# JessicaLeu-code/MotionPlanning_5D_m

Hardware: AMD Instinct MI355X
Metric: CFS iterations/sec, 5-DoF 30-wp 8-obs batch-1024; l_inf wp err vs quadprog (higher is better)
Workload: dtype f64

## Files before the change

### motionplanning_5d_m_amd/csrc/cfs_fused.hip

```cpp
#include "cfs_geom_dev.h"
#include <algorithm>
#include <atomic>

namespace {

#define STAMP(k) do { if (P.stamps) { const unsigned long long t_ = clock64(); if (tid == 0) s_acc[k] += t_ - t0_; t0_ = t_; } } while (0)

#ifndef CFS_CERT_AT
#define CFS_CERT_AT 6
#endif
constexpr int CERT_AT = CFS_CERT_AT;
#ifndef CFS_WG_PER_CU
#define CFS_WG_PER_CU 1
#endif
#ifndef CFS_ANGLE_ADD
#define CFS_ANGLE_ADD 0
#endif
#ifndef CFS_REF_A
#define CFS_REF_A 1e-4
#define CFS_REF_B 1e-9
#endif
#ifndef CFS_MV_BATCH
#define CFS_MV_BATCH 16
#endif
// ... 356 lines not shown
};
__host__ __device__ inline FusedLayout fused_layout(int NJ, int H, int nobs, int QB, int PR)
{
    FusedLayout L;
    const int HN = H * NJ, NS = 2 * NJ;
    int o = 0;
    L.rb = o; o += (int)(sizeof(DevRobot) / 8);
    L.ob = o; o += nobs * 6;
    L.x = o; o += H * NS;
    L.u = o; o += HN;
    L.qu = o; o += HN;
    L.g = o; o += nobs * HN;
    L.rhs = o; o += nobs * H;
    L.xs = o; o += 3 * HN;
    L.up = o; o += HN;
    L.act = o; o += (QB + 1) / 2;
    L.fre = o; o += (QB + 1) / 2;
    L.prev = o; o += (QB + 1) / 2;
    L.flag = o; o += (nobs * H + 4 * HN + 7) / 8;
    L.code = o; o += (nobs * H + 4 * HN + 1) / 2;
    L.red = o; o += 64;
    L.small = o; o += 4 * NJ + nobs;
    L.mx = o; o += HN;
    L.racc = o; o += HN;
    L.cost = o; o += (int)(sizeof(DevCost) / 8);
    o = (o + 1) & ~1;
    L.lin = o;
    L.wb = o; o += 3 * HN;
    L.zb = o; o += 3 * HN;
    L.d = o; o += QB;
    L.r = o; o += QB;
    L.rho = o; o += QB;
    L.lam = o; o += QB;
    L.prow = o; o += QB;
    L.slot = o; o += (nobs * H + 4 * HN + 3) / 4;
    L.ptail = o;
    o = (o + 1) & ~1;
    L.y = o;
    L.total_fixed = o;
    return L;
}

template <int NJ, int QB, bool IDENT>
__global__ __launch_bounds__(FT, CFS_WG_PER_CU) void CFS_FUSED_KERNEL(FusedParams P CFS_SOFT_KPARAM)
{
    constexpr int NS = 2 * NJ, NVT = nvt(NJ), NE = 2 * NJ + 1;
    extern __shared__ __attribute__((aligned(16))) double lds[];
    const int b = P.order ? P.order[blockIdx.x] : (int)blockIdx.x, tid = threadIdx.x;
    const int H = P.H, nobs = P.nobs, HN = H * NJ, nn = HN, NX = H * NS;
    const double dt = P.dt;
    constexpr int PR = QB < CFS_PR ? QB : CFS_PR;
    const FusedLayout L = fused_layout(NJ, H, nobs, QB, PR);
    DevRobot *rb = reinterpret_cast<DevRobot *>(lds + L.rb);
    double *s_ob = lds + L.ob, *s_x = lds + L.x, *s_u = lds + L.u, *s_qu = lds + L.qu, *s_g = lds + L.g;
    double *s_rhs = lds + L.rhs, *xs = lds + L.xs, *s_up = lds + L.up, *wb = lds + L.wb, *zb = lds + L.zb;
    double *s_d = lds + L.d, *s_r = lds + L.r, *s_rho = lds + L.rho, *s_lam = lds + L.lam, *s_prow = lds + L.prow;
    int *s_act = reinterpret_cast<int *>(lds + L.act);
    int *s_free = reinterpret_cast<int *>(lds + L.fre);
    int *s_prev = reinterpret_cast<int *>(lds + L.prev);
    unsigned char *s_flag = reinterpret_cast<unsigned char *>(lds + L.flag);
    unsigned short *s_slot = reinterpret_cast<unsigned short *>(lds + L.slot);
    int *s_code = reinterpret_cast<int *>(lds + L.code);
    double *red_base = lds + L.red;
    int red_sel = 0;
#define red (red_base + 24 * (red_sel ^= 1))
    double *s_lim = lds + L.small, *s_v0 = s_lim + NJ, *s_th0 = s_v0 + NJ, *s_margin = s_th0 + 2 * NJ;
    double *s_mx = lds + L.mx;
    double *s_racc = lds + L.racc;
    int pool_slot;
    {
        int *pubp = reinterpret_cast<int *>(red_base + 63);
        if (tid == 0) {
            int sidx = (int)(((blockIdx.x * 0x9E3779B1u) >> 8) % (unsigned)P.pool_n);
            int probes = 0;
            while (atomicCAS(&P.pool_flag[sidx * 16], 0, 1) != 0) {
                sidx = sidx + 1 == P.pool_n ? 0 : sidx + 1;
                __builtin_amdgcn_s_sleep(2);
                if (++probes > (1 << 22)) { sidx = -1; break; }
            }
            pubp[0] = sidx;
        }
        __syncthreads();
        pool_slot = pubp[0];
        if (pool_slot < 0) {
            if (tid == 0 && P.piece == 0) { P.status[b] = CFS_NUMERIC; P.iter_O[b] = 1; P.total_iter[b] = 0; }
            return;
        }
    }
    double *const s_pt = P.Pt + (size_t)pool_slot * P.pt_stride;
    double *s_Y = lds + L.y;
    const int QY = P.qy;
    double *const Yg = P.Yg + (size_t)pool_slot * nn * nn;
    auto drop_pool = [&]() {
        __syncthreads();
        if (tid == 0) { __threadfence(); atomicExch(&P.pool_flag[pool_slot * 16], 0); }
    };
    const int ncon = nobs * H + (P.has_bounds ? 4 : 2) * HN;
    const int maxit = 8 * nn + 200;
    for (int e = tid; e < ncon; e += FT) {
        int code;
        if (e < nobs * H) { const int j = e / H; code = mk_code(CT_COL, e - j * H, j); }
        else {
            const int f2 = e - nobs * H, ty = f2 / HN, k = f2 - ty * HN, i = k / NJ;
            code = mk_code(1 + ty, i, k - i * NJ);
        }
        s_code[e] = code;
    }

    {
        const double *src = reinterpret_cast<const double *>(P.rb);
        for (int e = tid; e < (int)(sizeof(DevRobot) / 8); e += FT) lds[L.rb + e] = src[e];
        for (int e = tid; e < nobs * 6; e += FT) s_ob[e] = P.obs[(size_t)b * nobs * 6 + e];
        for (int e = tid; e < NX; e += FT) s_x[e] = P.x_init[(size_t)b * NX + e];
        for (int e = tid; e < HN; e += FT) { s_u[e] = 0.0; s_qu[e] = 0.0; s_mx[e] = P.has_bounds ? P.maxin[e] : 0.0; }
        if (tid < NJ) {
            s_lim[tid] = P.lim[tid];
            s_v0[tid] = P.xR1[(size_t)b * NS + NJ + tid];
            s_th0[tid] = P.xR1[(size_t)b * NS + tid];
        }
        if (tid < nobs) s_margin[tid] = P.margin[tid];
        if (P.cost) {
            const double *csrc = reinterpret_cast<const double *>(P.cost);
            for (int e = tid; e < (int)(sizeof(DevCost) / 8); e += FT) lds[L.cost + e] = csrc[e];
        }
    }
    __syncthreads();
    if (P.has_bounds)
        for (int e = tid; e < HN; e += FT) {
            const int i = e / NJ, c = e - i * NJ;
            double acc = 0.0;
            for (int k = 0; k <= i; ++k) acc += ((double)(i - k) + 0.5) * s_mx[k * NJ + c];
            s_racc[e] = (dt * dt) * acc;
        }
    unsigned long long *s_acc = reinterpret_cast<unsigned long long *>(red_base + 48);
    if (tid < 12) s_acc[tid] = 0ull;
    unsigned long long t0_ = P.stamps ? clock64() : 0ull;
    double cost_new = P.caug[b], cost_old = 100000.0;
    int iter_O = 1, total_iter = 0, noise_row = 0, status = CFS_OK_MAXITER;
    bool done = false;
#if CFS_SOFT
    const double iw = S.inv_weight;
    int n_soft = 0;
    bool last_soft = false;
#endif
    const int nseg = nobs - P.nmesh;
    int launched = 0;
    if (P.resume) {
        for (int e = tid; e < NX; e += FT) s_x[e] = P.x_[(size_t)b * NX + e];
        for (int e = tid; e < HN; e += FT) { s_u[e] = P.u[(size_t)b * nn + e]; s_qu[e] = P.st_qu[(size_t)b * nn + e]; }
        cost_new = P.st_cost[2 * b]; cost_old = P.st_cost[2 * b + 1];
        iter_O = P.iter_O[b]; total_iter = P.total_iter[b]; status = P.status[b];
        noise_row = P.st_noise[b]; done = P.st_done[b] != 0;
        __syncthreads();
    } else if (P.piece == 0) {
        double d2 = 0.0;
        for (int e = tid; e < NX; e += FT) { const double v = s_x[e] - 1.0; d2 += v * v; }
        d2 = block_sum(d2, red, tid);
        if (sqrt(d2) < P.epsilon_O) { done = true; status = CFS_OK_CONVERGED; }
        else if (iter_O > P.max_o_iter) { done = true; status = CFS_OK_MAXITER; }
    } else if (P.piece == 2) {
        for (int e = tid; e < HN; e += FT) s_u[e] = P.u[(size_t)b * nn + e];
        __syncthreads();
    }

    PRow<PR, QB> Pr;
    int prev_q = 0;

    while (!done) {
        bool skip = false;
        if (P.piece == 0 && P.mode == CFS_MODE_PSGCFS) {
            skip = fabs(cost_new - cost_old) < 1e-4;
            if (!skip) cost_old = cost_new;
        } else if (P.piece == 0) cost_old = cost_new;
        const int noise_row_now = noise_row;
        if (P.piece == 0 && P.mode == CFS_MODE_PSGCFS && !skip) ++noise_row;
        auto prep = [&](int ph) {
            if (P.piece == 1) return;
            if (ph == 0) { for (int k = tid; k < HN; k += FT) xs[k] = s_u[k]; }
            else if (ph == 1) roll_lds<NJ>(xs, H, dt, tid);
            else if (ph == 2) {
                const bool psg = P.piece == 0 && P.mode == CFS_MODE_PSGCFS;
                const double sc = (double)iter_O * (double)iter_O + 1.0;
                const bool have = P.noise != nullptr && noise_row_now < P.noise_rows;
                for (int k = tid; k < HN; k += FT) {
                    s_up[k] = xs[2 * HN + k];
                    double v;
                    if (psg && skip) v = s_u[k];
                    else if (psg) {
                        const double nz = have ? P.noise[((size_t)b * P.noise_rows + noise_row_now) * nn + k] : 0.0;
                        v = s_u[k] - P.alpha * ((s_qu[k] + P.ff[(size_t)b * nn + k]) + 10.0 * nz / sc);
                    } else v = P.x0[(size_t)b * nn + k];
                    xs[k] = v;
                }
            } else roll_lds<NJ>(xs, H, dt, tid);
        };
        bool prepped = false;
#if CFS_JAC
        (void)NE;
        if (nseg > 0) {
            const int W = P.lin_w;
            double *s_sc = lds + L.lin;
            double *s_en = s_sc + W * NJ * 6;
            double *s_tw = s_en + W * NJ * 6;
            double *s_bd = s_en + W * NVT * 6;
            for (int w0 = 0; w0 < H; w0 += W) {
                const int Wc = min(W, H - w0);
                if (w0 == 0) prep(0);
                for (int e = tid; e < Wc * NJ; e += FT) {
                    const int m = e % NJ, wi = e / NJ;
                    double x = s_x[(w0 + wi) * NS + m];
                    x = x - rb->th_off[m];
                    double sn, cs;
                    sincos(x, &sn, &cs);
                    s_sc[e * 2] = sn;
                    s_sc[e * 2 + 1] = cs;
                }
                __syncthreads();
                for (int wi = tid; wi < Wc; wi += FT) arm_chain(rb, NJ, s_sc + wi * NJ * 2, s_en + wi * NJ * 6, s_tw + wi * NJ * 6);
                if (w0 == 0) prep(1);
                __syncthreads();
                STAMP(10);
                for (int e = tid; e < NJ * Wc * nseg; e += FT) {
                    const int j = e % nseg, wi = (e / nseg) % Wc, k0 = e / (nseg * Wc);
                    s_bd[(wi * NJ + k0) * nseg + j] = seg_seg_dist(s_en + (wi * NJ + k0) * 6, s_ob + j * 6);
                }
                if (w0 == 0) prep(2);
                __syncthreads();
                STAMP(0);
                for (int e = tid; e < Wc * nseg; e += FT) {
                    const int j = e % nseg, wi = e / nseg;
                    double m0 = INFINITY;
                    int lk = 0;
#pragma unroll
                    for (int k1 = 1; k1 <= NJ; ++k1) { const double bk = s_bd[(wi * NJ + k1 - 1) * nseg + j]; if (bk < m0) { m0 = bk; lk = k1; } }
                    if (P.dump_linkid && launched == 0) P.dump_linkid[((size_t)b * nobs + j) * H + w0 + wi] = lk;
                    s_rhs[j * H + w0 + wi] = m0;
                    double *g = s_g + (j * H + w0 + wi) * NJ;
                    if (lk > 0) winner_grad(s_en + (wi * NJ + lk - 1) * 6, s_tw + wi * NJ * 6, lk - 1, NJ, s_ob + j * 6, g);
                    else for (int m = 0; m < NJ; ++m) g[m] = 0.0;
                }
                if (w0 == 0) { prep(3); prepped = true; }
                if (w0 + W >= H) __syncthreads();
                STAMP(11);
            }
        }
#else
        if (nseg > 0) {
            const int W = P.lin_w;
            double *s_sc = lds + L.lin;
            double *s_en = s_sc + W * NJ * 6;
            double *s_bd = s_en + W * NVT * 6;
            double *s_dv = s_bd + W * NJ * nseg;
            unsigned short *s_list = reinterpret_cast<unsigned short *>(s_dv + W * nseg * NE);
            int *s_cnt = s_free;
            for (int w0 = 0; w0 < H; w0 += W) {
                const int Wc = min(W, H - w0);
                if (w0 == 0) prep(0);
#if CFS_ANGLE_ADD
                const double ch = cos(FD_EPS / 2), sh = sin(FD_EPS / 2);
                for (int e = tid; e < Wc * NJ; e += FT) {
                    const int m = e % NJ, wi = e / NJ;
                    double sn, cs;
                    sincos(s_x[(w0 + wi) * NS + m] - rb->th_off[m], &sn, &cs);
                    s_sc[e * 6] = sn;
                    s_sc[e * 6 + 1] = cs;
                    s_sc[e * 6 + 2] = sn * ch + cs * sh; s_sc[e * 6 + 3] = cs * ch - sn * sh;
                    s_sc[e * 6 + 4] = sn * ch - cs * sh; s_sc[e * 6 + 5] = cs * ch + sn * sh;
                }
#else
                for (int e = tid; e < Wc * NJ * 3; e += FT) {
                    const int var = e % 3, m = (e / 3) % NJ, wi = e / (3 * NJ);
                    double x = s_x[(w0 + wi) * NS + m];
                    if (var == 1) x = x + FD_EPS / 2;
                    else if (var == 2) x = x - FD_EPS / 2;
                    x = x - rb->th_off[m];
                    double sn, cs;
                    sincos(x, &sn, &cs);
                    s_sc[((wi * NJ + m) * 3 + var) * 2] = sn;
                    s_sc[((wi * NJ + m) * 3 + var) * 2 + 1] = cs;
                }
#endif
                __syncthreads();
                for (int e = tid; e < Wc * NE; e += FT) {
                    const int ev = e % NE, wi = e / NE;
                    double M[12], Mn[12], e6[6];
#pragma unroll
                    for (int k1 = 1; k1 <= NJ; ++k1) {
                        const int avar = (ev == 2 * k1 - 1) ? 1 : (ev >= 2 * k1 ? 2 : 0);
                        const double sn = s_sc[((wi * NJ + k1 - 1) * 3 + avar) * 2], cs = s_sc[((wi * NJ + k1 - 1) * 3 + avar) * 2 + 1];
                        fk_step(rb, k1 - 1, sn, cs, k1 == 1 ? nullptr : M, Mn);
#pragma unroll
                        for (int qq = 0; qq < 12; ++qq) M[qq] = Mn[qq];
                        if (ev <= 2 * k1) {
                            link_ends(rb, k1 - 1, M, e6);
                            double *dstE = s_en + (wi * NVT + kvoff(k1) + ev) * 6;
#pragma unroll
                            for (int qq = 0; qq < 6; ++qq) dstE[qq] = e6[qq];
                        }
                    }
                }
                if (w0 == 0) prep(1);
                __syncthreads();
                STAMP(10);
#if CFS_LIN_UNROLL
#pragma unroll 2
#endif
                for (int e = tid; e < NJ * Wc * nseg; e += FT) {
                    const int j = e % nseg, wi = (e / nseg) % Wc, k0 = e / (nseg * Wc);
                    s_bd[(wi * NJ + k0) * nseg + j] = seg_seg_dist(s_en + (wi * NVT + kvoff(k0 + 1)) * 6, s_ob + j * 6);
                }
                if (tid < NJ) s_cnt[tid] = 0;
                if (w0 == 0) prep(2);
                __syncthreads();
                for (int e = tid; e < Wc * nseg; e += FT) {
                    const int j = e % nseg, wi = e / nseg;
                    double bk[NJ], m0 = INFINITY;
                    int lk = 0;
#pragma unroll
                    for (int k1 = 1; k1 <= NJ; ++k1) { bk[k1 - 1] = s_bd[(wi * NJ + k1 - 1) * nseg + j]; if (bk[k1 - 1] < m0) { m0 = bk[k1 - 1]; lk = k1; } }
                    if (P.dump_linkid && launched == 0) P.dump_linkid[((size_t)b * nobs + j) * H + w0 + wi] = lk;
                    const double thr = P.no_prune ? INFINITY : fmax(m0, 0.0001) + rb->prune_tol;
#pragma unroll
                    for (int k1 = 1; k1 <= NJ; ++k1)
                        if (bk[k1 - 1] < thr) s_list[(k1 - 1) * W * nseg + atomicAdd(&s_cnt[k1 - 1], 1)] = (unsigned short)((wi << 8) | j);
                    s_dv[e * NE] = m0;
#pragma unroll
                    for (int ev = 1; ev < NE; ++ev) s_dv[e * NE + ev] = INFINITY;
                }
                if (w0 == 0) { prep(3); prepped = true; }
                __syncthreads();
                STAMP(0);
                {
                    int offs[NJ + 1];
                    offs[0] = 0;
#pragma unroll
                    for (int k1 = 1; k1 <= NJ; ++k1) offs[k1] = offs[k1 - 1] + s_cnt[k1 - 1] * 2 * k1;
#if CFS_LIN_UNROLL
#pragma unroll 2
#endif
                    for (int e = tid; e < offs[NJ]; e += FT) {
                        int k1 = 1, ent = 0, v = 1;
#pragma unroll
                        for (int kk = 1; kk <= NJ; ++kk)
                            if (e >= offs[kk - 1] && e < offs[kk]) {
                                const int r_ = e - offs[kk - 1];
                                k1 = kk; ent = r_ / (2 * kk); v = r_ - ent * (2 * kk) + 1;
                            }
                        const int item = s_list[(k1 - 1) * W * nseg + ent], wi = item >> 8, j = item & 255;
                        const double dis = seg_seg_dist(s_en + (wi * NVT + kvoff(k1) + v) * 6, s_ob + j * 6);
                        double *dv = s_dv + (wi * nseg + j) * NE;
                        const int evhi = (v == 2 * k1) ? NE - 1 : v;
                        for (int ev = v; ev <= evhi; ++ev)
                            __hip_atomic_fetch_min(dv + ev, dis, __ATOMIC_RELAXED, __HIP_MEMORY_SCOPE_WORKGROUP);
                    }
                }
                __syncthreads();
                STAMP(11);
                for (int e = tid; e < Wc * nseg; e += FT) {
                    const int j = e % nseg, wi = e / nseg;
                    double dev[NE];
#pragma unroll
                    for (int ev = 0; ev < NE; ++ev) dev[ev] = s_dv[e * NE + ev];
                    s_rhs[j * H + w0 + wi] = dev[0];
#pragma unroll
                    for (int m = 0; m < NJ; ++m) s_g[(j * H + w0 + wi) * NJ + m] = (dev[2 * m + 1] - dev[2 * m + 2]) / FD_EPS;
                }
                if (w0 + W >= H) __syncthreads();
            }
        }
#endif
        if (!prepped && P.piece != 1) {
            prep(0); __syncthreads(); prep(1); __syncthreads(); prep(2); __syncthreads(); prep(3); __syncthreads();
        }

        if (P.nmesh > 0) {
            for (int e = tid; e < P.nmesh * H; e += FT) s_rhs[nseg * H + e] = P.ext_dist[(size_t)b * P.nmesh * H + e];
            for (int e = tid; e < P.nmesh * HN; e += FT) s_g[nseg * HN + e] = P.ext_grad[(size_t)b * P.nmesh * HN + e];
            __syncthreads();
        }

        if (P.dump_dist && launched == 0) {
            for (int e = tid; e < nobs * H; e += FT) P.dump_dist[(size_t)b * nobs * H + e] = s_rhs[e];
            for (int e = tid; e < nobs * HN; e += FT) P.dump_grad[(size_t)b * nobs * HN + e] = s_g[e];
        }
        if (P.piece == 1) { drop_pool(); return; }

        STAMP(0);
        int qp_status = QP_OK, iters = 0;
        int qhi = 0, nfree = 0;
        int npolish = 0;
        auto n_combine = [&](const double *coef, const double *base, int pc_) {
            const int ptype_ = pc_ >> 16, pi_ = (pc_ >> 8) & 0xff, pj_ = pc_ & 0xff;
            const bool two = H <= 32;
            const int lane = two ? (tid & 31) : (tid & 63);
            const int iR = H - 1 - lane;
            const int cstep = two ? 2 * (FT / 64) : FT / 64;
            for (int c = two ? (tid >> 5) : (tid >> 6); c < NJ; c += cstep) {
                double Rp = 0.0, Rv = 0.0;
                if (lane < H) {
                    const int sp_ = s_slot[nobs * H + iR * NJ + c], sm_ = s_slot[nobs * H + HN + iR * NJ + c];
                    for (int j0 = 0; j0 < nobs; j0 += 8) {
                        int sl[8];
#pragma unroll
                        for (int jj = 0; jj < 8; ++jj) sl[jj] = j0 + jj < nobs ? s_slot[(j0 + jj) * H + iR] : 0;
#pragma unroll
                        for (int jj = 0; jj < 8; ++jj)
                            if (sl[jj]) Rp += coef[sl[jj] - 1] * s_g[((j0 + jj) * H + iR) * NJ + c];
                    }
                    if (sp_) Rv -= dt * coef[sp_ - 1];
                    if (sm_) Rv += dt * coef[sm_ - 1];
                }
                const double S1 = two ? half_scan_incl(Rp) : wave_scan_incl(Rp);
                const double cmb = (dt * dt) * S1 + Rv;
                const double S2V = two ? half_scan_incl(cmb) : wave_scan_incl(cmb);
                const double nr_rev = S2V - (0.5 * dt * dt) * S1;
                const int src = (lane < H ? H - 1 - lane : lane) + (two ? (tid & 32) : 0);
                const double nr = __shfl(nr_rev, src, 64);
                double z0 = 0.0;
                if (lane < H) {
                    if (base) z0 = base[lane * NJ + c];
                    else if (ptype_ == CT_COL) z0 = lane <= pi_ ? s_g[(pj_ * H + pi_) * NJ + c] * ((dt * dt) * ((double)(pi_ - lane) + 0.5)) : 0.0;
                    else z0 = (c == pj_ && lane <= pi_) ? (ptype_ == CT_VELP ? -dt : dt) : 0.0;
                    z0 -= nr;
                }
                const double sv = dt * (two ? half_scan_incl(z0) : wave_scan_incl(z0));
                const double spo = dt * (two ? half_scan_incl(sv) : wave_scan_incl(sv)) - (0.5 * dt) * sv;
                if (lane < H) { zb[lane * NJ + c] = z0; zb[HN + lane * NJ + c] = sv; zb[2 * HN + lane * NJ + c] = spo; }
            }
        };
        auto y_combine = [&](const double *coef, const double *base) {
            const int qa = min(qhi, QY);
            for (int k = tid; k < HN; k += FT) {
                double z0 = base ? base[k] : 0.0, z1 = 0.0, z2 = 0.0, z3 = 0.0;
                int a = 0;
                for (; a + 4 <= qa; a += 4) {
                    z0 -= coef[a] * s_Y[a * HN + k];
                    z1 -= coef[a + 1] * s_Y[(a + 1) * HN + k];
                    z2 -= coef[a + 2] * s_Y[(a + 2) * HN + k];
                    z3 -= coef[a + 3] * s_Y[(a + 3) * HN + k];
                }
                for (; a < qa; ++a) z0 -= coef[a] * s_Y[a * HN + k];
                for (a = qa; a + CFS_TU <= qhi; a += CFS_TU) {
                    double t[CFS_TU];
#pragma unroll
                    for (int jj = 0; jj < CFS_TU; ++jj) t[jj] = Yg[(size_t)(a + jj) * nn + k];
#pragma unroll
                    for (int jj = 0; jj < CFS_TU; jj += 4) {
                        z0 -= coef[a + jj] * t[jj]; z1 -= coef[a + jj + 1] * t[jj + 1]; z2 -= coef[a + jj + 2] * t[jj + 2]; z3 -= coef[a + jj + 3] * t[jj + 3];
                    }
                }
                for (; a < qhi; ++a) z0 -= coef[a] * Yg[(size_t)a * nn + k];
                zb[k] = (z0 + z1) + (z2 + z3);
            }
        };
        auto y_combine_roll = [&](const double *coef, const double *base) {
            const int lane = tid & 31;
            for (int c = tid >> 5; c < NJ; c += 2 * (FT / 64)) {
                const int k = lane * NJ + c;
                double z0 = 0.0, z1 = 0.0, z2 = 0.0, z3 = 0.0;
                if (lane < H) {
                    z0 = base ? base[k] : 0.0;
                    int a = 0;
                    for (; a + 4 <= qhi; a += 4) {
                        z0 -= coef[a] * s_Y[a * HN + k];
                        z1 -= coef[a + 1] * s_Y[(a + 1) * HN + k];
                        z2 -= coef[a + 2] * s_Y[(a + 2) * HN + k];
                        z3 -= coef[a + 3] * s_Y[(a + 3) * HN + k];
                    }
                    for (; a < qhi; ++a) z0 -= coef[a] * s_Y[a * HN + k];
                }
                const double z = (z0 + z1) + (z2 + z3);
                const double sv = dt * half_scan_incl(z);
                const double spo = dt * half_scan_incl(sv) - (0.5 * dt) * sv;
                if (lane < H) { zb[k] = z; zb[HN + k] = sv; zb[2 * HN + k] = spo; }
            }
        };
        auto gather_w = [&](int code) {
            const int ptype_ = code >> 16, pi_ = (code >> 8) & 0xff, pj_ = code & 0xff;
            for (int k = tid; k < HN; k += FT) {
                double w0, w1, w2;
                if (ptype_ == CT_COL) {
                    w0 = w1 = w2 = 0.0;
#pragma unroll
                    for (int cs = 0; cs < NJ; ++cs) {
                        const double gc = s_g[(pj_ * H + pi_) * NJ + cs];
                        const size_t o = (size_t)(pi_ * NJ + cs) * nn + k;
                        w0 += gc * P.M1[o];
                        if (!(P.opt & 1)) { w1 += gc * P.M1v[o]; w2 += gc * P.M1p[o]; }
                    }
                } else {
                    const bool vel = ptype_ == CT_VELP || ptype_ == CT_VELM;
                    const double sg = (ptype_ == CT_VELP || ptype_ == CT_BNDP) ? -1.0 : 1.0;
                    const size_t o = (size_t)(pi_ * NJ + pj_) * nn + k;
                    w0 = sg * (vel ? P.M2 : P.M3)[o];
                    w1 = w2 = 0.0;
                    if (!(P.opt & 1)) { w1 = sg * (vel ? P.M2v : P.M3v)[o]; w2 = sg * (vel ? P.M2p : P.M3p)[o]; }
                }
                wb[k] = w0; wb[HN + k] = w1; wb[2 * HN + k] = w2;
            }
        };
#if CFS_SOFT
        bool soft = false;
        double viol = 0.0;
#endif
        if (!skip) {
            for (int e = tid; e < ncon; e += FT) { s_flag[e] = 0; s_slot[e] = 0; }
            Pr.zero(s_pt, tid, 0);
            if (tid < QB) { s_prev[tid] = s_act[tid]; s_d[tid] = 0.0; s_r[tid] = 0.0; s_rho[tid] = 0.0; s_prow[tid] = 0.0; s_lam[tid] = 0.0; s_act[tid] = -1; }
            for (int e = tid; e < nobs * H; e += FT) {
                const int j = e / H, i = e - j * H;
                double gp = 0.0;
#pragma unroll
                for (int c = 0; c < NJ; ++c) gp += s_g[e * NJ + c] * s_up[i * NJ + c];
                s_rhs[e] = (s_rhs[e] - s_margin[j]) - gp;
            }
            double fgain = 0.0, fbound;
            {
                double p0 = 0.0, p1 = 0.0, p2 = 0.0, p3 = 0.0;
                for (int k = tid; k < HN; k += FT) {
                    const int c = k % NJ;
                    const double rb_ = P.has_bounds ? s_mx[k] : (2.0 * s_lim[c] + fabs(s_v0[c])) / dt;
                    const double rs_ = s_lim[c] + fabs(s_v0[c]);
                    p0 += rb_ * rb_;
                    p1 += xs[k] * xs[k];
                    p2 += rs_ * rs_;
                    p3 += xs[HN + k] * xs[HN + k];
                }
                block_sum4(p0, p1, p2, p3, red, tid);
                const double lmax = P.lmax_H;
                const double ru = sqrt(p0) + sqrt(p1), rs = sqrt(p2) + sqrt(p3);
                fbound = 1.0001 * 0.5 * fmin(lmax * ru * ru, P.lmax_vel * rs * rs);
            }
            const bool cert_on = !(P.opt & 16) && nobs > 1;
            auto certificate = [&]() -> bool {
                int hit = 0;
                for (int e = tid; e < H * nobs; e += FT) {
                    const int i = e / nobs, a = e - i * nobs;
                    double ga[NJ], cen[NJ], rad[NJ], na2 = 0.0;
#pragma unroll
                    for (int c = 0; c < NJ; ++c) { ga[c] = s_g[(a * H + i) * NJ + c]; na2 += ga[c] * ga[c]; }
                    if (!(na2 > 0.0)) continue;
                    const double ia = 1.0 / sqrt(na2), ra = -s_rhs[a * H + i] * ia;
#pragma unroll
                    for (int c = 0; c < NJ; ++c) {
                        const double f = dt * ((double)i + 0.5);
                        double lo = f * (-s_lim[c] - s_v0[c]), hi = f * (s_lim[c] - s_v0[c]);
                        if (P.has_bounds) { lo = fmax(lo, -s_racc[i * NJ + c]); hi = fmin(hi, s_racc[i * NJ + c]); }
                        cen[c] = 0.5 * (lo + hi); rad[c] = fmax(0.5 * (hi - lo), 0.0);
                    }
                    for (int b2 = a + 1; b2 < nobs; ++b2) {
                        double gb[NJ], nb2 = 0.0;
#pragma unroll
                        for (int c = 0; c < NJ; ++c) { gb[c] = s_g[(b2 * H + i) * NJ + c]; nb2 += gb[c] * gb[c]; }
                        if (!(nb2 > 0.0)) continue;
                        const double ib = 1.0 / sqrt(nb2), rb = -s_rhs[b2 * H + i] * ib;
#pragma unroll
                        for (int wk = 0; wk < 3; ++wk) {
                            const double w = wk == 0 ? 1.0 : (wk == 1 ? 0.5 : 2.0);
                            double lhs = 0.0, mag = 0.0;
#pragma unroll
                            for (int c = 0; c < NJ; ++c) {
                                const double cc = ga[c] * ia + w * (gb[c] * ib);
                                lhs += cc * cen[c] + fabs(cc) * rad[c];
                                mag += fabs(cc) * (fabs(cen[c]) + rad[c]);
                            }
                            const double rhs_ = ra + w * rb;
                            if (lhs < rhs_ - 1e-9 * (1.0 + fabs(rhs_) + mag)) hit = 1;
                        }
                    }
                    if (i + 1 < H)
                        for (int b2 = 0; b2 < nobs; ++b2) {
                            double gb[NJ], nb2 = 0.0;
#pragma unroll
                            for (int c = 0; c < NJ; ++c) { gb[c] = s_g[(b2 * H + i + 1) * NJ + c]; nb2 += gb[c] * gb[c]; }
                            if (!(nb2 > 0.0)) continue;
                            const double ib = 1.0 / sqrt(nb2), rb = -s_rhs[b2 * H + i + 1] * ib;
#pragma unroll
                            for (int wk = 0; wk < 3; ++wk) {
                                const double w = wk == 0 ? 1.0 : (wk == 1 ? 0.5 : 2.0);
                                double lhs = 0.0, mag = 0.0;
#pragma unroll
                                for (int c = 0; c < NJ; ++c) {
                                    const double cb = w * (gb[c] * ib), cc = ga[c] * ia + cb;
                                    lhs += (cc * cen[c] + fabs(cc) * rad[c]) + (cb * (-dt * s_v0[c]) + fabs(cb) * (dt * s_lim[c]));
                                    mag += fabs(cc) * (fabs(cen[c]) + rad[c]) + fabs(cb) * dt * (fabs(s_v0[c]) + s_lim[c]);
                                }
                                const double rhs_ = ra + w * rb;
                                if (lhs < rhs_ - 1e-9 * (1.0 + fabs(rhs_) + mag)) hit = 1;
                            }
                        }
                }
                return block_sum((double)hit, red, tid) > 0.0;
            };
            STAMP(1);
#if CFS_SOFT
          int iters_hard = 0;
          for (;;) {
            if (soft) {
                iters_hard = iters; iters = 0;
                __syncthreads();
                for (int e = tid; e < ncon; e += FT) { s_flag[e] = 0; s_slot[e] = 0; }
                Pr.zero(s_pt, tid, 0);
                if (tid < QB) { s_d[tid] = 0.0; s_r[tid] = 0.0; s_rho[tid] = 0.0; s_prow[tid] = 0.0; s_lam[tid] = 0.0; s_act[tid] = -1; }
                qhi = 0; nfree = 0; npolish = 0; qp_status = QP_OK; fgain = 0.0;
                __syncthreads();
                prep(0); __syncthreads(); prep(1); __syncthreads(); prep(2); __syncthreads(); prep(3); __syncthreads();
            }
#endif
            if (IF_HARD(P.piece == 0) && !(P.opt & 8) && prev_q > 0 && prev_q <= min(64, P.warm_max > 0 ? P.warm_max : min(PR, IDENT ? 64 : 24))) {
                int *pub = reinterpret_cast<int *>(red_base + 62);
                int q = 0;
                for (int s0 = 0; s0 < (IDENT ? 1 : prev_q); ++s0) {
                    int c_all = -1;
                    if (!IDENT) {
                        c_all = s_prev[s0];
                        if (c_all < 0) continue;
                        gather_w(c_all);
                        __syncthreads();
                        if (P.opt & 1) { roll_lds<NJ>(wb, H, dt, tid); __syncthreads(); }
                    }
                if (tid < 64) {
                    for (int s1 = IDENT ? 0 : s0; s1 < (IDENT ? prev_q : s0 + 1); ++s1) {
                        const int c = s_prev[s1];
                        if (c < 0) continue;
                        const int mine = tid < q ? s_act[tid] : -1;
                        const double dv = mine >= 0 ? (IDENT ? gram_ident<NJ>(mine, c, s_g, H, dt) : ndot<NJ>(mine, wb, s_g, H)) : 0.0;
                        s_d[tid] = dv;
                        const double spp_ = IDENT ? gram_ident<NJ>(c, c, s_g, H, dt) : ndot<NJ>(c, wb, s_g, H);
                        if (!IDENT && tid == 0) pub[0] = 0;
                        sync_rows(true);
                        const double rv = mine >= 0 ? Pr.dot(s_d, s_pt, tid, q) : 0.0;
                        const double delta_ = spp_ - wave_add(dv * rv);
                        if (!(delta_ > 1e-6 * spp_)) { sync_rows(true); continue; }
                        const int slot = q, qn = q + 1;
                        const double inv = 1.0 / delta_;
                        s_r[tid] = tid == slot ? -1.0 : rv;
                        if (slot >= PR) s_pt[(slot - PR) * QB + tid] = 0.0;
                        sync_rows(true);
                        if (tid < q) Pr.axpy(rv * inv, s_r, s_pt, tid, qn);
                        else if (tid == slot) Pr.set_scaled(-inv, s_r, s_pt, tid, qn);
                        if (tid == 0) {
                            const int ct = c >> 16, ci = (c >> 8) & 0xff, cj = c & 0xff;
                            const int cidx = ct == CT_COL ? cj * H + ci : nobs * H + (ct - 1) * HN + ci * NJ + cj;
                            s_act[slot] = c; s_flag[cidx] = 1; s_slot[cidx] = (unsigned short)(slot + 1);
                            if (!IDENT) pub[0] = 1;
                        }
                        if (IDENT) q = qn;
                        sync_rows(true);
                    }
                }
                    if (!IDENT) {
                        __syncthreads();
                        if (pub[0]) {
                            if (q < QY) { for (int k = tid; k < HN; k += FT) s_Y[q * HN + k] = wb[k]; }
                            else { for (int k = tid; k < HN; k += FT) Yg[(size_t)q * nn + k] = wb[k]; }
                            ++q;
                        }
                    }
                }
                if (tid < 64) {
                    int nf = 0;
                    double lamv = 0.0, s0v = 0.0;
                    bool ok = true;
                    for (int round = 0;; ++round) {
                        const int mine = tid < q ? s_act[tid] : -1;
                        double bb;
                        s0v = mine >= 0 ? slack_of<NJ>(mine, xs, s_g, s_rhs, s_lim, s_v0, s_mx, H, &bb) : 0.0;
                        s_d[tid] = s0v;
// ... 540 lines not shown
```

Measured before the change: 5.823 million.

## Replace per-ev atomic min fan-out with tail buffer and prefix-min reconstruction

The dense link-distance loop now advances its (j, wi, k0) indices incrementally with carries, which removes the per-iteration integer divides and modulos. In the pruned finite-difference pass, a link-end variant (v == 2k) that used to issue an atomic min on every later slot now issues a single atomic min into a per-link tail slot, reusing s_bd reset to infinity. The gradient pass rebuilds the later slots from a running prefix minimum over those tail slots. This cuts the number of LDS atomics, at the cost of extra s_bd writes and reads.

```diff
diff --git a/motionplanning_5d_m_amd/csrc/cfs_fused.hip b/motionplanning_5d_m_amd/csrc/cfs_fused.hip
--- a/motionplanning_5d_m_amd/csrc/cfs_fused.hip
+++ b/motionplanning_5d_m_amd/csrc/cfs_fused.hip
@@ -682,12 +682,23 @@
                 if (w0 == 0) prep(1);
                 __syncthreads();
                 STAMP(10);
+                {
+                    const int fq = FT / nseg, fj = FT - fq * nseg, fk = fq / Wc, fw = fq - fk * Wc;
+                    int j = tid % nseg, wi = tid / nseg, k0 = wi / Wc;
+                    wi -= k0 * Wc;
 #if CFS_LIN_UNROLL
 #pragma unroll 2
 #endif
-                for (int e = tid; e < NJ * Wc * nseg; e += FT) {
-                    const int j = e % nseg, wi = (e / nseg) % Wc, k0 = e / (nseg * Wc);
-                    s_bd[(wi * NJ + k0) * nseg + j] = seg_seg_dist(s_en + (wi * NVT + kvoff(k0 + 1)) * 6, s_ob + j * 6);
+                    for (int e = tid; e < NJ * Wc * nseg; e += FT) {
+                        s_bd[(wi * NJ + k0) * nseg + j] = seg_seg_dist(s_en + (wi * NVT + kvoff(k0 + 1)) * 6, s_ob + j * 6);
+                        j += fj;
+                        const int cj = j >= nseg;
+                        if (cj) j -= nseg;
+                        wi += fw + cj;
+                        const int cw = wi >= Wc;
+                        if (cw) wi -= Wc;
+                        k0 += fk + cw;
+                    }
                 }
                 if (tid < NJ) s_cnt[tid] = 0;
                 if (w0 == 0) prep(2);
@@ -701,8 +712,10 @@
                     if (P.dump_linkid && launched == 0) P.dump_linkid[((size_t)b * nobs + j) * H + w0 + wi] = lk;
                     const double thr = P.no_prune ? INFINITY : fmax(m0, 0.0001) + rb->prune_tol;
 #pragma unroll
-                    for (int k1 = 1; k1 <= NJ; ++k1)
+                    for (int k1 = 1; k1 <= NJ; ++k1) {
                         if (bk[k1 - 1] < thr) s_list[(k1 - 1) * W * nseg + atomicAdd(&s_cnt[k1 - 1], 1)] = (unsigned short)((wi << 8) | j);
+                        s_bd[(wi * NJ + k1 - 1) * nseg + j] = INFINITY;
+                    }
                     s_dv[e * NE] = m0;
 #pragma unroll
                     for (int ev = 1; ev < NE; ++ev) s_dv[e * NE + ev] = INFINITY;
@@ -728,10 +741,8 @@
                             }
                         const int item = s_list[(k1 - 1) * W * nseg + ent], wi = item >> 8, j = item & 255;
                         const double dis = seg_seg_dist(s_en + (wi * NVT + kvoff(k1) + v) * 6, s_ob + j * 6);
-                        double *dv = s_dv + (wi * nseg + j) * NE;
-                        const int evhi = (v == 2 * k1) ? NE - 1 : v;
-                        for (int ev = v; ev <= evhi; ++ev)
-                            __hip_atomic_fetch_min(dv + ev, dis, __ATOMIC_RELAXED, __HIP_MEMORY_SCOPE_WORKGROUP);
+                        double *dst = v == 2 * k1 ? s_bd + (wi * NJ + k1 - 1) * nseg + j : s_dv + (wi * nseg + j) * NE + v;
+                        __hip_atomic_fetch_min(dst, dis, __ATOMIC_RELAXED, __HIP_MEMORY_SCOPE_WORKGROUP);
                     }
                 }
                 __syncthreads();
@@ -742,8 +753,13 @@
 #pragma unroll
                     for (int ev = 0; ev < NE; ++ev) dev[ev] = s_dv[e * NE + ev];
                     s_rhs[j * H + w0 + wi] = dev[0];
-#pragma unroll
-                    for (int m = 0; m < NJ; ++m) s_g[(j * H + w0 + wi) * NJ + m] = (dev[2 * m + 1] - dev[2 * m + 2]) / FD_EPS;
+                    double tl = INFINITY;
+#pragma unroll
+                    for (int m = 0; m < NJ; ++m) {
+                        const double dp = fmin(dev[2 * m + 1], tl);
+                        tl = fmin(tl, s_bd[(wi * NJ + m) * nseg + j]);
+                        s_g[(j * H + w0 + wi) * NJ + m] = (dp - fmin(dev[2 * m + 2], tl)) / FD_EPS;
+                    }
                 }
                 if (w0 + W >= H) __syncthreads();
             }
```

After: 5.851 million (median of 6 runs). Within noise of the previous version (+0.5%).
